# prashantraina/neural_raytracing

Hardware: NVIDIA B200
Metric: rays_per_sec (higher is better)
Workload: dtype f16

## Files before the change

### neural_raytracing_b200/csrc/nrt_tc.cu

```cuda
#include <stdlib.h>

#include "tc_core.cuh"
#include "camera_math.cuh"

namespace tc {

template <int IN, int LAT, int OUT>
struct IoPlain {
  const float* x; const float* latent; float* out; int out_act;
  __device__ __forceinline__ void load(int64_t m, float* v) const {
#pragma unroll
    for (int j = 0; j < IN; ++j) v[j] = __ldg(x + m * IN + j);
#pragma unroll
    for (int j = 0; j < LAT; ++j) v[IN + j] = __ldg(latent + m * LAT + j);
  }
  __device__ __forceinline__ void store(int64_t m, const float* o) const {
#pragma unroll
    for (int j = 0; j < OUT; ++j) {
      float v = o[j];
      if (out_act == NRT_OUT_SIGMOID) v = 1.0f / (1.0f + __expf(-v));
      else if (out_act == NRT_OUT_SOFTPLUS) v = v > 20.0f ? v : __logf(1.0f + __expf(v));
      else if (out_act == NRT_OUT_TANH) v = tanhf(v);
      out[m * OUT + j] = v;
    }
// ... 69 lines not shown
    }
  }
  __device__ __forceinline__ void load(int64_t m, float* v) const {
    const int64_t ray = ray_of(m, S, s_shift);
    if (lat32) {
      const float4* src = reinterpret_cast<const float4*>(latent) + (m >> 7) * (int64_t)(NLAT / 4 * 128) + (m & 127);
#pragma unroll
      for (int j = 0; j < NLAT / 4; ++j) {
        const float4 q = __ldg(src + j * 128);
        v[4 * j] = q.x; v[4 * j + 1] = q.y; v[4 * j + 2] = q.z; v[4 * j + 3] = q.w;
      }
    } else {
      const uint4* src = reinterpret_cast<const uint4*>(latent) + (m >> 7) * (int64_t)(NLAT / 8 * 128) + (m & 127);
#pragma unroll
      for (int j = 0; j < NLAT / 8; ++j) {
        const uint4 q = __ldg(src + j * 128);
        const uint32_t w[4] = {q.x, q.y, q.z, q.w};
#pragma unroll
        for (int e = 0; e < 4; ++e) {
          if (fmt == 0) {
            v[8 * j + 2 * e] = Elem<0>::back((uint16_t)(w[e] & 0xffff)); v[8 * j + 2 * e + 1] = Elem<0>::back((uint16_t)(w[e] >> 16));
          } else {
            v[8 * j + 2 * e] = Elem<1>::back((uint16_t)(w[e] & 0xffff)); v[8 * j + 2 * e + 1] = Elem<1>::back((uint16_t)(w[e] >> 16));
          }
        }
      }
    }
    const int view = dir_and_view(ray, v + NLAT);
#pragma unroll
    for (int j = 0; j < LD; ++j) v[NLAT + 3 + j] = __ldg(light_code + (int64_t)view * LD + j);
  }
  static constexpr int kPackedPairs = PACKED ? NLAT / 2 : 0;
  __device__ __forceinline__ void load_packed(int64_t m, uint32_t* w, float* v) const {
    const int64_t ray = ray_of(m, S, s_shift);
    const uint4* src = reinterpret_cast<const uint4*>(latent) + (m >> 7) * (int64_t)(NLAT / 8 * 128) + (m & 127);
#pragma unroll
    for (int j = 0; j < NLAT / 8; ++j) {
      const uint4 q = __ldg(src + j * 128);
      w[4 * j] = q.x; w[4 * j + 1] = q.y; w[4 * j + 2] = q.z; w[4 * j + 3] = q.w;
    }
    const int view = dir_and_view(ray, v + NLAT);
#pragma unroll
    for (int j = 0; j < LD; ++j) v[NLAT + 3 + j] = __ldg(light_code + (int64_t)view * LD + j);
  }
  __device__ __forceinline__ void store(int64_t m, const float* o) const {
#pragma unroll
    for (int j = 0; j < 3; ++j) {
      float v = o[j];
      if (out_act == NRT_OUT_SIGMOID) v = 1.0f / (1.0f + __expf(-v));
      else if (out_act == NRT_OUT_TANH) v = tanhf(v);
      rgb[m * 3 + j] = v;
    }
  }
};

static long long* g_dbg_timeline = nullptr;
extern "C" void nrtdbg_set_timeline(long long* dev_buf) { g_dbg_timeline = dev_buf; }

#ifndef NRT_SPH_MAX
#define NRT_SPH_MAX 128
#endif
constexpr int kSphMax = NRT_SPH_MAX;
__device__ __forceinline__ float* sph_table() {
  __shared__ __align__(16) float tab[kSphMax * 13];
  return tab;
}
__device__ __forceinline__ void sph_fill(const SdfDev& sd) {
  if (sd.n > kSphMax) return;
  float* tab = sph_table();
  for (int e = threadIdx.x; e < sd.n * 13; e += blockDim.x) {
    const int i = e / 13, k = e - i * 13;
    float v;
    if (k == 12) v = __ldg(sd.radii + i);
    else {
// ... 149 lines not shown
  __device__ __forceinline__ void store(int64_t m, const float* o) const {
    float p[3];
    point(m, p);
    val[m] = sphere_smin_fast<true>(sd, p[0], p[1], p[2]) + o[0];
  }
};
__global__ void k_scan_argmin(const float* __restrict__ val, const float* __restrict__ rays, int64_t R, int n1, double step,
                              int32_t* __restrict__ best_idx, float* __restrict__ best_pos, float* __restrict__ min_val) {
  const int lane = threadIdx.x & 31;
  const int64_t r = ((int64_t)blockIdx.x * blockDim.x + threadIdx.x) >> 5;
  if (r >= R) return;
  const float* v = val + r * n1;
  float best = 3.0e38f;
  int idx = 0x7fffffff;
  for (int k = lane; k < n1; k += 32) {
    const float x = v[k];
    if (x < best) { best = x; idx = k; }
  }
  for (int o = 16; o > 0; o >>= 1) {
    const float ob = __shfl_xor_sync(0xffffffffu, best, o);
    const int oi = __shfl_xor_sync(0xffffffffu, idx, o);
    if (ob < best || (ob == best && oi < idx)) { best = ob; idx = oi; }
  }
  if (lane == 0) {
    best_idx[r] = idx;
    if (min_val) min_val[r] = best;
    const float tb = __fmul_rn((float)idx, (float)step);
    for (int j = 0; j < 3; ++j) best_pos[r * 3 + j] = __fadd_rn(rays[r * 6 + j], __fmul_rn(tb, rays[r * 6 + 3 + j]));
  }
}

template <class NET, class IO, int FMT, class SV = NoSave>
static int launch(const void* blob, const IO& io, int64_t M, cudaStream_t st, int tag = TAG_TC_MLP, SV sv = SV{}) {
  const size_t bytes = (size_t)NET::SMEM_BYTES + 256;
  auto kern = k_mlp_tc<NET, IO, FMT, SV>;
  NRT_CUDA(cudaFuncSetAttribute(kern, cudaFuncAttributeMaxDynamicSharedMemorySize, (int)bytes));
  const int64_t ntiles = (M + 127) / 128;
  const int grid = (int)std::min<int64_t>((ntiles + NET::NSLOT - 1) / NET::NSLOT, (int64_t)nrt_sm_count());
  NrtProfScope _ps(tag, st);
  kern<<<grid, NET::threads(NET::WPS), bytes, st>>>(reinterpret_cast<const uint8_t*>(blob) + NET::BLOB_OFF, io, M, g_dbg_timeline, sv);
  NRT_CUDA(cudaGetLastError());
  return NRT_OK;
}

using NetNerfFirst = Net<3, 0, 16, 128, 5, 3, 65, NRT_ACT_LEAKY_RELU>;
using NetNerfFirstR = Net<3, 0, 16, 128, 5, 3, 65, NRT_ACT_LEAKY_RELU, (NRT_BIAS_MMA & 4) != 0>;
using NetNerfSecondPT = Net<70, 0, 16, 64, 8, 3, 3, NRT_ACT_LEAKY_RELU>;
using NetNerfSecondLE = Net<115, 0, 16, 64, 8, 3, 3, NRT_ACT_LEAKY_RELU>;
using NetNeuralBsdf = Net<3, 0, 64, 96, 6, 3, 3, NRT_ACT_LEAKY_RELU>;
using NetOcc = Net<5, 0, 16, 64, 8, 3, 1, NRT_ACT_LEAKY_RELU>;
using NetPlainFirst = Net<3, 32, 16, 32, 5, 3, 33, NRT_ACT_LEAKY_RELU>;
using NetPlainSecond = Net<2, 64, 16, 32, 5, 3, 3, NRT_ACT_LEAKY_RELU>;
using NetSdfShift = Net<3, 0, 32, 128, 8, 3, 1, NRT_ACT_SOFTPLUS>;

template <class NET>
static bool matches(const MlpDev& d) {
  return d.in_size == NET::IN && d.latent == NET::LAT && d.freqs == NET::F && d.hidden == NET::H && d.L == NET::L &&
         d.skip == NET::SKIP && d.out == NET::OUT && d.act == NET::ACT;
}
template <class NET>
static bool matches(const nrt_mlp_t& m) {
  return m.in_size == NET::IN && m.latent_size == NET::LAT && m.freqs == NET::F && m.hidden == NET::H && m.num_layers == NET::L &&
         m.skip == NET::SKIP && m.out_size == NET::OUT && m.act == NET::ACT;
}

}

using namespace tc;

static int fmt_of(int prec) { return prec == NRT_PREC_BF16 ? 1 : 0; }

extern "C" int64_t nrt_mlp_tc_blob_bytes(const nrt_mlp_t* m, int prec) {
  NRT_REQUIRE(m != nullptr, "mlp descriptor is NULL");
  NRT_REQUIRE(prec == NRT_PREC_F16 || prec == NRT_PREC_BF16, "nrt_mlp_tc_blob_bytes: prec must be F16 or BF16");
  NRT_REQUIRE(m->num_layers >= 1 && m->num_layers <= NRT_MAX_LAYERS && m->hidden % 16 == 0, "unsupported MLP shape");
  if (matches<NetNerfFirst>(*m)) return (int64_t)NetNerfFirstR::BLOB_OFF + NetNerfFirstR::Y.bytes;
  const Layout y = make_layout(m->in_size, m->latent_size, m->freqs, m->hidden, m->num_layers, m->skip, m->out_size);
  return (int64_t)y.bytes;
}

extern "C" int nrt_mlp_pack_tc(const nrt_mlp_t* m, int prec, void* blob_out, void* stream) {
// ... 234 lines not shown
```

### neural_raytracing_b200/csrc/tc_core.cuh

```cuda
#pragma once
#include <cuda_bf16.h>
#include <cuda_fp16.h>

#include <algorithm>
#include <type_traits>

#include "nrt_common.cuh"

namespace tc {

constexpr int kMaxOps = NRT_MAX_LAYERS + 3;

struct Layout {
  int split, XR, KRAW, KE, KX, KPH, FP, NOP;
  int n_ops;
  int opN[kMaxOps], opK[kMaxOps];
  int op_off[kMaxOps];
  int w_elems;
  int bias_off[kMaxOps];
  int bias_floats;
  int wout_f32_off;
  int basis_f32_off;
  int bytes;
};
// ... 673 lines not shown
          for (int i = 0; i < 8; ++i) q[i] = fmaf(q[i], u[i], 9.974489612e-01f);
#pragma unroll
          for (int i = 0; i < 8; ++i) a[i] = fmaf(q[i], u[i], fmaxf(a[i], 0.0f));
        } else {
#pragma unroll
          for (int i = 0; i < 8; ++i) u[i] = lg2_approx(1.0f + u[i]);
#pragma unroll
          for (int i = 0; i < 8; ++i) a[i] = fmaf(0.6931471805599453f, u[i], fmaxf(a[i], 0.0f));
        }
      } else {
#pragma unroll
        for (int i = 0; i < 8; ++i) a[i] = fmaxf(a[i], 0.01f * a[i]);
      }
#pragma unroll
      for (int i = 0; i < 8; ++i) {
        const float4 w = *reinterpret_cast<const float4*>(wout + (32 * c + 8 * g + i) * 4);
        o[0] = fmaf(a[i], w.x, o[0]);
        if constexpr (OUT > 1) o[1] = fmaf(a[i], w.y, o[1]);
        if constexpr (OUT > 2) o[2] = fmaf(a[i], w.z, o[2]);
        if constexpr (OUT > 3) o[3] = fmaf(a[i], w.w, o[3]);
      }
      if constexpr (SAVE) {
#pragma unroll
        for (int i = 0; i < 4; ++i) pk[4 * g + i] = Elem<FMT>::pack(a[2 * i], a[2 * i + 1]);
      }
    }
    if constexpr (SAVE) {
      save_cols<16>(save_row, 32 * c, pk);
      mask_ptr[(int64_t)c * mask_stride] = sign_mask32(pk);
    }
    if (c + 1 < NC) tc_wait_ld();
  }
  if constexpr (SAVE) save_row[tile_elem(H)] = one16<FMT>();
}

template <int ACT, int FMT, int H>
__device__ __forceinline__ void convert_row_savef32(uint32_t dD, uint32_t aU, float* __restrict__ acts, int64_t stride) {
  constexpr int NC = H / 32;
  uint32_t buf[2][32];
  TmemIO<32>::ld(dD, buf[0]);
  tc_wait_ld();
#pragma unroll
  for (int c = 0; c < NC; ++c) {
    if (c + 1 < NC) TmemIO<32>::ld(dD + 32 * (c + 1), buf[(c + 1) & 1]);
    uint32_t pk[16];
    convert32<ACT, FMT>(buf[c & 1], pk);
    TmemIO<16>::st(aU + 16 * c, pk);
    if (acts != nullptr) {
#pragma unroll
      for (int i = 0; i < 16; ++i) {
        acts[(int64_t)(32 * c + 2 * i) * stride] = Elem<FMT>::back((uint16_t)(pk[i] & 0xffffu));
        acts[(int64_t)(32 * c + 2 * i + 1) * stride] = Elem<FMT>::back((uint16_t)(pk[i] >> 16));
      }
    }
    if (c + 1 < NC) tc_wait_ld();
  }
}
template <int ACT, int FMT, int H, int OUT>
__device__ __forceinline__ void convert_row_out_savef32(uint32_t dD, const float* __restrict__ wout, float* __restrict__ o,
                                                        float* __restrict__ acts, int64_t stride) {
  constexpr int NC = H / 32;
  uint32_t buf[2][32];
  TmemIO<32>::ld(dD, buf[0]);
  tc_wait_ld();
#pragma unroll
  for (int c = 0; c < NC; ++c) {
// ... 158 lines not shown
  __syncwarp();
}
template <class NET, int FMT, int PART = 0, bool BMMA = false, int ZLO = 0>
__device__ __forceinline__ void issue_stage_dyn(int st, uint32_t b_addr, uint32_t dD, uint32_t aU, uint32_t aE,
                                                uint64_t* done_bar) {
#define NRT_STAGE_CASE(S) case S: if constexpr (S < NET::STAGES && (PART == 0 || S >= 2)) issue_stage<NET, FMT, S, PART, BMMA, ZLO>(b_addr, dD, aU, aE, done_bar); break;
  switch (st) {
    NRT_STAGE_CASE(0) NRT_STAGE_CASE(1) NRT_STAGE_CASE(2) NRT_STAGE_CASE(3) NRT_STAGE_CASE(4) NRT_STAGE_CASE(5)
    NRT_STAGE_CASE(6) NRT_STAGE_CASE(7) NRT_STAGE_CASE(8) NRT_STAGE_CASE(9) NRT_STAGE_CASE(10) NRT_STAGE_CASE(11)
    NRT_STAGE_CASE(12) NRT_STAGE_CASE(13) NRT_STAGE_CASE(14) NRT_STAGE_CASE(15) NRT_STAGE_CASE(16) NRT_STAGE_CASE(17)
    NRT_STAGE_CASE(18) NRT_STAGE_CASE(19) NRT_STAGE_CASE(20) NRT_STAGE_CASE(21) NRT_STAGE_CASE(22)
    default: break;
  }
#undef NRT_STAGE_CASE
}
__device__ __forceinline__ void stream_op(uint8_t* dst, const uint8_t* src, uint32_t bytes, uint64_t* bar) {
  mbar_expect_tx(bar, bytes);
  for (uint32_t off = 0; off < bytes; off += 32768u) bulk_g2s(dst + off, src + off, min(32768u, bytes - off), bar);
}

template <class T, class = void> struct PackedPairsOf { static constexpr int value = 0; };
template <class T> struct PackedPairsOf<T, std::void_t<decltype(T::kPackedPairs)>> { static constexpr int value = T::kPackedPairs; };
template <class T, class = void> struct HasCtaInit : std::false_type {};
template <class T> struct HasCtaInit<T, std::void_t<decltype(&T::cta_init)>> : std::true_type {};
template <class T, class = void> struct IsIterative : std::false_type {};
template <class T> struct IsIterative<T, std::void_t<typename T::State>> : std::true_type {};
struct NoState {};
template <class T, class = void> struct StateOf { using type = NoState; };
template <class T> struct StateOf<T, std::void_t<typename T::State>> { using type = typename T::State; };

__device__ __forceinline__ void named_bar_sync(int id, int nthreads) {
  asm volatile("bar.sync %0, %1;" ::"r"(id), "r"(nthreads) : "memory");
}

#ifdef NRT_MAXNREG
#define NRT_KMLP_BOUNDS(T) __maxnreg__(((65536 / (T)) / 8 * 8) > 255 ? 255 : ((65536 / (T)) / 8 * 8))
#else
#define NRT_KMLP_BOUNDS(T) __launch_bounds__(T, 1)
#endif
template <class NET, class IO, int FMT, class SV = NoSave, int WPS = NET::WPS>
__global__ void NRT_KMLP_BOUNDS(NET::threads(WPS))
k_mlp_tc(const uint8_t* __restrict__ blob, IO io, int64_t M, long long* __restrict__ dbg, SV sv = SV{}) {
  constexpr int EPI = WPS * 32;
  static_assert(NET::FITS_TMEM, "network does not fit in TMEM");
  static_assert(NET::FITS_SMEM, "stage buffers do not fit in shared memory");
  constexpr int kDbgIt0 = 4, kDbgIts = 4;
  auto stamp = [&](int it, int st, int slot, int k) {
    if (dbg != nullptr && slot < 2 && blockIdx.x == 0 && it >= kDbgIt0 && it < kDbgIt0 + kDbgIts)
      dbg[(((it - kDbgIt0) * NET::STAGES + st) * 2 + slot) * 8 + k] = clock64();
  };
  using E = Elem<FMT>;
  constexpr Layout Y = NET::Y;
  constexpr int H = NET::H, IN = NET::IN, LAT = NET::LAT, F = NET::F, L = NET::L;
  constexpr int NSLOT = NET::NSLOT;
  extern __shared__ __align__(128) uint8_t smem[];
  constexpr bool STREAM = NET::STREAM;
  uint16_t* sW = reinterpret_cast<uint16_t*>(smem);
  const float* sBias = reinterpret_cast<const float*>(smem + (STREAM ? (size_t)NSLOT * 2 * NET::MAXOP : (size_t)Y.w_elems * 2));
  __shared__ __align__(8) uint64_t bar_w;
  __shared__ __align__(8) uint64_t bar_wfull[3][2];
  __shared__ uint32_t s_opoff[NET::STAGES], s_opbytes[NET::STAGES];
  __shared__ __align__(8) uint64_t bar_ready[3];
  __shared__ __align__(8) uint64_t bar_ready_a[3];
  __shared__ __align__(8) uint64_t bar_done[3];
  constexpr bool KSPLIT = NET::KSPLIT && WPS == 4 && !SV::kOn && !SV::kF32;
#ifndef NRT_SOFTPLUS_FULLROW
#define NRT_SOFTPLUS_FULLROW 0
#endif
#ifndef NRT_SOFTPLUS_PIPE
#define NRT_SOFTPLUS_PIPE 1
#endif
  constexpr bool kPipeRow = NRT_SOFTPLUS_PIPE != 0 && SoftplusOf<IO>::value != 0 && NET::ACT == NRT_ACT_SOFTPLUS && !KSPLIT &&
                            !SV::kOn && !SV::kF32;
  constexpr bool kFullRow = NRT_SOFTPLUS_FULLROW != 0 && !kPipeRow && NET::ACT == NRT_ACT_SOFTPLUS && !KSPLIT && !SV::kOn && !SV::kF32;
  __shared__ uint32_t tmem_base_s;
  __shared__ uint32_t s_bias[NET::STAGES];
  constexpr bool ITER = IsIterative<IO>::value;
  constexpr bool BMMA = NET::BIAS_MMA && !KSPLIT && WPS == 4 && !SV::kOn && !SV::kF32;
  static_assert(BMMA || !NET::BIAS_ROWS, "the render layout has no fp32 biases to pre-load");
  constexpr int kPP = (!ITER && !NET::SPLIT && !SV::kOn && !SV::kF32 && LAT == 0 && NET::ACT == NRT_ACT_LEAKY_RELU) ? PackedPairsOf<IO>::value : 0;
  constexpr int ZLO = (NRT_BIAS_MMA & 2) ? 2 * kPP / 16 : 0;
  __shared__ volatile uint32_t s_slot_live[3];
  __shared__ uint32_t s_warp_live[3][4];

  const int tid = threadIdx.x;
  const int warp = tid >> 5;
  constexpr bool SELF = NET::SELF;
  const int mma_id = SELF ? -1 : warp - NET::NWG * WPS;
  const bool is_mma_warp = SELF ? warp == 0 : mma_id == 0;
  __shared__ uint32_t s_issue_lock;
  const int64_t ntiles = (M + 127) / 128;
  if constexpr (HasCtaInit<IO>::value) io.cta_init();
  if (tid < NET::STAGES) {
    s_bias[tid] = (uint32_t)Y.bias_off[tid];
    s_opoff[tid] = (uint32_t)Y.op_off[tid] * 2;
    s_opbytes[tid] = (uint32_t)(Y.opN[tid] * Y.opK[tid] * 2);
  }

  if (tid == 0) {
    s_slot_live[0] = 1; s_slot_live[1] = 1; s_slot_live[2] = 1;
    s_issue_lock = 0;
    mbar_init(&bar_w, 1);
    for (int s = 0; s < 3; ++s) {
      mbar_init(&bar_ready[s], EPI); mbar_init(&bar_done[s], 1); mbar_init(&bar_ready_a[s], EPI);
      mbar_init(&bar_wfull[s][0], 1); mbar_init(&bar_wfull[s][1], 1);
    }
    asm volatile("fence.mbarrier_init.release.cluster;" ::: "memory");
  }
  __syncthreads();
  if (is_mma_warp) {
    asm volatile("tcgen05.alloc.cta_group::1.sync.aligned.shared::cta.b32 [%0], 512;" ::"r"(smem_u32(&tmem_base_s)) : "memory");
    asm volatile("tcgen05.relinquish_alloc_permit.cta_group::1.sync.aligned;" ::: "memory");
    if ((tid & 31) == 0) {
      if (STREAM) {
        mbar_expect_tx(&bar_w, (uint32_t)NET::BIAS_BYTES);
        bulk_g2s(smem + (size_t)NSLOT * 2 * NET::MAXOP, blob + (size_t)Y.w_elems * 2, (uint32_t)NET::BIAS_BYTES, &bar_w);
      } else {
        mbar_expect_tx(&bar_w, (uint32_t)Y.bytes);
        constexpr uint32_t kChunk = 32768;
        for (uint32_t off = 0; off < (uint32_t)Y.bytes; off += kChunk) {
          const uint32_t n = min(kChunk, (uint32_t)Y.bytes - off);
          bulk_g2s(smem + off, blob + off, n, &bar_w);
        }
      }
    }
  }
  tc_fence_before();
  __syncthreads();
  tc_fence_after();
  if (tmem_base_s != 0u) __trap();
  constexpr uint32_t tmem = 0u;
  if constexpr (BMMA) {
    if (warp < 4) {
      const uint32_t one = (uint32_t)one16<FMT>();
      const uint32_t r[8] = {one | (one << 16), one, 0u, 0u, 0u, 0u, 0u, 0u};
      TmemIO<8>::st(tmem + ((uint32_t)(warp * 32) << 16) + (uint32_t)NET::ONES_COL, r);
      tc_wait_st();
    }
    tc_fence_before();
    __syncthreads();
    tc_fence_after();
  }
  mbar_wait(&bar_w, 0);

  if (mma_id >= 0) {
    constexpr int NMMA = NET::NMMA;
    constexpr bool OWN = NMMA == NSLOT;
    auto mine = [&](int slot) { return slot % (NMMA > 0 ? NMMA : 1) == mma_id; };
#ifndef NRT_MMA_ALTERNATE
#define NRT_MMA_ALTERNATE 0
#endif
    constexpr bool ALT = NRT_MMA_ALTERNATE != 0 && !OWN && NSLOT == 2 && !KSPLIT;
    int turn = 0;
    bool live[3];
    auto is_ready = [&](int slot, uint64_t* bar, uint32_t parity) {
      if constexpr (OWN) { mbar_wait(bar, parity); return true; }
      else if constexpr (ALT) {
        if (slot != turn && live[turn]) return false;
        mbar_wait(bar, parity);
        turn = slot ^ 1;
        return true;
      }
      else return mbar_test(bar, parity);
    };
    const uint32_t sW_addr = smem_u32(sW);
    int st[3] = {NET::FIRST_STAGE, NET::FIRST_STAGE, NET::FIRST_STAGE};
    uint32_t n_ready[3] = {0, 0, 0};
    uint32_t n_ready_a[3] = {0, 0, 0};
    bool half_issued[3] = {false, false, false};
    int64_t tile[3] = {(int64_t)blockIdx.x * NSLOT, (int64_t)blockIdx.x * NSLOT + 1, (int64_t)blockIdx.x * NSLOT + 2};
    live[0] = mine(0) && (ITER || tile[0] < ntiles);
    live[1] = NSLOT > 1 && mine(1) && (ITER || tile[1] < ntiles);
    live[2] = NSLOT > 2 && mine(2) && (ITER || tile[2] < ntiles);
    int it_dbg[3] = {0, 0, 0};
    uint32_t n_issued[3] = {0, 0, 0};
    if (STREAM) {
#pragma unroll
      for (int slot = 0; slot < NSLOT; ++slot)
        if (live[slot] && elect_one())
          stream_op(smem + (size_t)(slot * 2) * NET::MAXOP, blob + s_opoff[NET::FIRST_STAGE], s_opbytes[NET::FIRST_STAGE],
                    &bar_wfull[slot][0]);
      __syncwarp();
    }
    while (live[0] || live[1] || live[2]) {
      bool progressed = false;
#pragma unroll
      for (int slot = 0; slot < NSLOT; ++slot) {
        if (!live[slot]) continue;
        if constexpr (KSPLIT) {
          if (st[slot] >= 2 && !half_issued[slot]) {
            if (!is_ready(slot, &bar_ready_a[slot], n_ready_a[slot] & 1)) continue;
            progressed = true;
            n_ready_a[slot]++;
            half_issued[slot] = true;
            tc_fence_after();
            const uint32_t base = tmem + slot * NET::COLS;
            uint32_t b_addr = sW_addr;
            if (STREAM) {
              const uint32_t b = n_issued[slot] & 1;
              mbar_wait(&bar_wfull[slot][b], (n_issued[slot] >> 1) & 1);
              b_addr = sW_addr + (uint32_t)((slot * 2 + b) * NET::MAXOP);
            }
            if ((tid & 31) == 0) stamp(it_dbg[slot], st[slot], slot, 0);
            issue_stage_dyn<NET, FMT, 1>(st[slot], b_addr, base, base + NET::DC, base + NET::DC + NET::UC, &bar_done[slot]);
            continue;
          }
        }
        if (!is_ready(slot, &bar_ready[slot], n_ready[slot] & 1)) continue;
        progressed = true;
        n_ready[slot]++;
        tc_fence_after();
        if constexpr (ITER) {
          if (st[slot] == NET::FIRST_STAGE && s_slot_live[slot] == 0) {
            live[slot] = false;
            if (STREAM) mbar_wait(&bar_wfull[slot][n_issued[slot] & 1], (n_issued[slot] >> 1) & 1);
            continue;
          }
        }
        if ((tid & 31) == 0) stamp(it_dbg[slot], st[slot], slot, 1);
        const uint32_t base = tmem + slot * NET::COLS;
        uint32_t b_addr = sW_addr;
        if (STREAM) {
          const uint32_t b = n_issued[slot] & 1;
          mbar_wait(&bar_wfull[slot][b], (n_issued[slot] >> 1) & 1);
          b_addr = sW_addr + (uint32_t)((slot * 2 + b) * NET::MAXOP);
          if ((tid & 31) == 0) stamp(it_dbg[slot], st[slot], slot, 0);
        }
        if (KSPLIT && half_issued[slot]) {
          half_issued[slot] = false;
          issue_stage_dyn<NET, FMT, 2>(st[slot], b_addr, base, base + NET::DC, base + NET::DC + NET::UC, &bar_done[slot]);
        } else {
          issue_stage_dyn<NET, FMT, 0, BMMA, ZLO>(st[slot], b_addr, base, base + NET::DC, base + NET::DC + NET::UC, &bar_done[slot]);
        }
        if ((tid & 31) == 0) stamp(it_dbg[slot], st[slot], slot, 2);
        if (++st[slot] == NET::END_STAGE) {
          st[slot] = NET::FIRST_STAGE;
          it_dbg[slot]++;
          if constexpr (!ITER) {
            tile[slot] += (int64_t)gridDim.x * NSLOT;
            live[slot] = tile[slot] < ntiles;
          }
        }
        if (STREAM) {
          n_issued[slot]++;
          if (live[slot] && elect_one()) {
            const uint32_t nb = n_issued[slot] & 1;
            stream_op(smem + (size_t)(slot * 2 + nb) * NET::MAXOP, blob + s_opoff[st[slot]], s_opbytes[st[slot]],
                      &bar_wfull[slot][nb]);
          }
          __syncwarp();
        }
      }
#ifndef NRT_MMA_POLL_SLEEP_NS
#define NRT_MMA_POLL_SLEEP_NS 0
#endif
      if (NRT_MMA_POLL_SLEEP_NS > 0 && !progressed) __nanosleep(NRT_MMA_POLL_SLEEP_NS);
    }
  } else {
    const int slot = warp / WPS;
    const int half = (WPS == 8) ? ((warp >> 2) & 1) : 0;
    const bool primary = half == 0;
    const int lane_row = (warp & 3) * 32 + (tid & 31);
    constexpr int HW = (WPS == 8) ? H / 2 : H;
    if (slot < NSLOT) {
      const uint32_t lane_off = ((uint32_t)((warp & 3) * 32)) << 16;
      const uint32_t base = tmem + slot * NET::COLS + lane_off;
      const uint32_t dD = base, aU = base + NET::DC, aE = base + NET::DC + NET::UC;
      uint32_t n_done = 0;
      int it_dbg = 0;
#ifndef NRT_DBG_LANE
#define NRT_DBG_LANE 0
#endif
      auto estamp = [&](int st, int k) { if (lane_row == NRT_DBG_LANE) stamp(it_dbg, st, slot, k); };
      typename StateOf<IO>::type state;
      if constexpr (ITER) io.init(state);
      const bool leader = SELF && (warp % WPS) == 0;
      int st_mma = NET::FIRST_STAGE;
      uint32_t n_ready_l = 0, n_issued_l = 0;
      const uint32_t sW_addr_l = smem_u32(sW);
      if constexpr (SELF) {
        if (leader) {
          if (elect_one())
            stream_op(smem + (size_t)(slot * 2) * NET::MAXOP, blob + s_opoff[NET::FIRST_STAGE], s_opbytes[NET::FIRST_STAGE],
                      &bar_wfull[slot][0]);
          __syncwarp();
        }
      }
      auto self_issue = [&]() {
        if constexpr (SELF) {
          if (leader) {
            mbar_wait(&bar_ready[slot], n_ready_l & 1); n_ready_l++;
            const uint32_t b = n_issued_l & 1;
            mbar_wait(&bar_wfull[slot][b], (n_issued_l >> 1) & 1);
            if ((tid & 31) == 0) {
              while (atomicCAS(&s_issue_lock, 0u, 1u) != 0u) __nanosleep(64);
            }
            __syncwarp();
            tc_fence_after();
            if ((tid & 31) == 0) stamp(it_dbg, st_mma, slot, 1);
            const uint32_t base0 = tmem + slot * NET::COLS;
            issue_stage_dyn<NET, FMT>(st_mma, sW_addr_l + (uint32_t)((slot * 2 + b) * NET::MAXOP), base0, base0 + NET::DC,
                                      base0 + NET::DC + NET::UC, &bar_done[slot]);
            if ((tid & 31) == 0) {
              stamp(it_dbg, st_mma, slot, 2);
              __threadfence_block();
              atomicExch(&s_issue_lock, 0u);
            }
            if (++st_mma == NET::END_STAGE) st_mma = NET::FIRST_STAGE;
            n_issued_l++;
            if (elect_one()) {
              const uint32_t nb = n_issued_l & 1;
              stream_op(smem + (size_t)(slot * 2 + nb) * NET::MAXOP, blob + s_opoff[st_mma], s_opbytes[st_mma], &bar_wfull[slot][nb]);
            }
            __syncwarp();
          }
        }
      };
      auto self_drain = [&]() {
        if constexpr (SELF) {
          if (leader) mbar_wait(&bar_wfull[slot][n_issued_l & 1], (n_issued_l >> 1) & 1);
        }
      };
#ifndef NRT_SLOT_STAGGER
#define NRT_SLOT_STAGGER 900
#endif
      if (NRT_SLOT_STAGGER > 0 && slot > 0) {
        const long long t_start = clock64();
        while (clock64() - t_start < (long long)slot * NRT_SLOT_STAGGER) {}
      }
      for (int64_t t0 = (int64_t)blockIdx.x * NSLOT;; t0 += (int64_t)gridDim.x * NSLOT, ++it_dbg) {
        int64_t m = 0;
        bool valid;
        float x[IN + LAT];
        uint32_t pw[kPP > 0 ? kPP : 1];
        if constexpr (ITER) {
          valid = primary ? io.next(state, x) : false;
          const unsigned bal = __ballot_sync(0xffffffffu, valid);
          if (primary && (tid & 31) == 0) s_warp_live[slot][warp & 3] = bal;
          named_bar_sync(1 + slot, EPI);
          const bool any = (s_warp_live[slot][0] | s_warp_live[slot][1] | s_warp_live[slot][2] | s_warp_live[slot][3]) != 0;
          if (!any) {
            if (lane_row == 0) s_slot_live[slot] = 0;
            mbar_arrive(&bar_ready[slot]);
            self_drain();
            break;
          }
        } else {
          const int64_t tile = t0 + slot;
          if (tile >= ntiles) { self_drain(); break; }
          m = tile * 128 + lane_row;
          valid = m < M;
          if constexpr (kPP > 0) {
            if (valid && primary) io.load_packed(m, pw, x);
          } else {
            if (valid && primary) io.load(m, x);
          }
        }
        if (!primary) {
          if constexpr (!NET::ENC_CUDA) {
            mbar_arrive(&bar_ready[slot]);
            mbar_wait(&bar_done[slot], n_done & 1); n_done++;
          }
          mbar_arrive(&bar_ready[slot]);
          self_issue();
        } else {
        uint32_t ex[NET::XR / 2];
        {
          if (!valid) {
#pragma unroll
            for (int j = 0; j < IN + LAT; ++j) x[j] = 0.0f;
          }
          uint32_t ax[NET::KX / 2];
#pragma unroll
          for (int j = 0; j < NET::KX / 2; ++j) { ax[j] = 0; ex[j] = 0; }
          if constexpr (NET::SPLIT) {
            uint16_t v[16];
#pragma unroll
            for (int j = 0; j < 16; ++j) v[j] = 0;
            uint16_t a[2 * IN];
#pragma unroll
            for (int j = 0; j < IN; ++j) {
              const uint16_t hi = E::cvt(x[j]);
              const uint16_t lo = E::cvt(x[j] - E::back(hi));
              v[j] = hi; v[IN + j] = lo; v[2 * IN + j] = hi;
              const float ax_ = act_fast<NET::ACT>(x[j]);
              const uint16_t ahi = E::cvt(ax_);
              a[j] = ahi; a[IN + j] = E::cvt(ax_ - E::back(ahi));
            }
            if constexpr (NET::BIAS_ROWS) {
#pragma unroll
              for (int t = 0; t < 3; ++t) v[NET::BR.row + t] = one16<FMT>();
            }
#pragma unroll
            for (int j = 0; j < 8; ++j) ax[j] = (uint32_t)v[2 * j] | ((uint32_t)v[2 * j + 1] << 16);
#pragma unroll
            for (int j = 0; j < IN; ++j) ex[j] = (uint32_t)a[2 * j] | ((uint32_t)a[2 * j + 1] << 16);
            if constexpr (NET::BIAS_ROWS) {
#pragma unroll
              for (int t = 0; t < 3; ++t) ex[(NET::BR.row + t) / 2] |= (uint32_t)one16<FMT>() << (16 * ((NET::BR.row + t) & 1));
            }
// ... 19 lines not shown
            }
            if constexpr (NET::INPLACE) { tmem_store<NET::XR / 2>(aE, ax); tmem_store<NET::XR / 2>(aU, lx); }
            else { tmem_store<NET::XR / 2>(aU, ax); tmem_store<NET::XR / 2>(aE, lx); }
          }
          if constexpr (SV::kOn) {
            static_assert(!ITER, "activation tiles are saved by the tile policies only");
            uint16_t* rr = tile_row_ptr(sv.enc_raw, m >> 7, NET::KE + kTileRowsExtra, lane_row);
            uint16_t* ra = tile_row_ptr(sv.enc_act, m >> 7, NET::KE + kTileRowsExtra, lane_row);
            save_cols<NET::KX / 2>(rr, 0, ax);
            if constexpr (!NET::INPLACE) save_cols<NET::XR / 2>(ra, 0, ex);
            rr[tile_elem(NET::KE)] = one16<FMT>();
            ra[tile_elem(NET::KE)] = one16<FMT>();
          }
          if constexpr (LAT > 0) {
            uint32_t lr[LAT / 2], la[LAT / 2];
#pragma unroll
            for (int j = 0; j < LAT / 2; ++j) {
              lr[j] = E::pack(x[IN + 2 * j], x[IN + 2 * j + 1]);
              la[j] = E::pack(act_fast<NET::ACT>(x[IN + 2 * j]), act_fast<NET::ACT>(x[IN + 2 * j + 1]));
            }
            tmem_store<LAT / 2>(aU + (NET::XR + 2 * F) / 2, lr);
            tmem_store<LAT / 2>(aE + (NET::XR + 2 * F) / 2, la);
            if constexpr (SV::kOn) {
              save_cols<LAT / 2>(tile_row_ptr(sv.enc_raw, m >> 7, NET::KE + kTileRowsExtra, lane_row), NET::XR + 2 * F, lr);
              save_cols<LAT / 2>(tile_row_ptr(sv.enc_act, m >> 7, NET::KE + kTileRowsExtra, lane_row), NET::XR + 2 * F, la);
            }
          }
          if constexpr (!NET::ENC_CUDA) {
            tc_wait_st();
            tc_fence_before();
            mbar_arrive(&bar_ready[slot]);
          }
        }
        {
          uint32_t ph[F];
          if constexpr (NET::ENC_CUDA) {
            const float* sB = sBias + Y.basis_f32_off;
#pragma unroll
            for (int f = 0; f < F; ++f) {
              float p = x[0] * sB[f];
#pragma unroll
              for (int j = 1; j < IN; ++j) p = fmaf(x[j], sB[j * NET::FP + f], p);
              ph[f] = __float_as_uint(p);
            }
          } else {
            mbar_wait(&bar_done[slot], n_done & 1); n_done++;
            tc_fence_after();
            tmem_load<F>(dD, ph);
            tc_wait_ld();
            if constexpr (!NET::INPLACE) tmem_store<NET::XR / 2>(aE, ex);
          }
          if constexpr (!BMMA) preload_bias<H>(dD, sBias + s_bias[1]);
          uint32_t sr[F / 2], cr[F / 2], sa[F / 2], ca[F / 2];
#pragma unroll
          for (int j = 0; j < F / 2; ++j) {
            float s0, c0, s1, c1;
            sincos_fast(__uint_as_float(ph[2 * j]), &s0, &c0);
            sincos_fast(__uint_as_float(ph[2 * j + 1]), &s1, &c1);
            sr[j] = E::pack(s0, s1); cr[j] = E::pack(c0, c1);
            sa[j] = E::pack(act_fast<NET::ACT>(s0), act_fast<NET::ACT>(s1));
            ca[j] = E::pack(act_fast<NET::ACT>(c0), act_fast<NET::ACT>(c1));
          }
          if constexpr (NET::INPLACE) {
            tmem_store<F / 2>(aE + NET::XR / 2, sr);
            tmem_store<F / 2>(aE + NET::XR / 2 + F / 2, cr);
          } else {
            tmem_store<F / 2>(aU + NET::XR / 2, sr);
// ... 55 lines not shown
            long long* d = nullptr;
            if (dbg != nullptr && lane_row == 0 && slot < 2 && blockIdx.x == 0 && it_dbg >= kDbgIt0 && it_dbg < kDbgIt0 + kDbgIts)
              d = dbg + (((it_dbg - kDbgIt0) * NET::STAGES + 2 + st) * 2 + slot) * 8;
            convert_row_split<NET::ACT, FMT, HW>(dD, aU, &bar_ready_a[slot], &bar_ready[slot], pre, d ? d + 5 : nullptr,
                                                 d ? d + 6 : nullptr);
            estamp(2 + st, 7);
          } else {
          if constexpr (SV::kOn)
            convert_row<NET::ACT, FMT, HW, true>(dD + coff, aU + coff / 2,
                tile_row_ptr(sv.acts, (int64_t)st * sv.ntiles + (m >> 7), H + kTileRowsExtra, lane_row), coff, primary ? H : -1,
                sv.masks + (int64_t)st * (H / 32) * (sv.ntiles * 128) + m, sv.ntiles * 128);
          else if constexpr (SV::kF32)
            convert_row_savef32<NET::ACT, FMT, HW>(dD + coff, aU + coff / 2,
                                                   valid ? sv.acts + ((int64_t)st * H) * sv.M + m : nullptr, sv.M);
          else if constexpr (kPipeRow) {
            long long* d = nullptr;
#ifdef NRT_DBG_CONV
            if (dbg != nullptr && lane_row == NRT_DBG_LANE && slot < 2 && blockIdx.x == 0 && it_dbg >= kDbgIt0 && it_dbg < kDbgIt0 + kDbgIts)
              d = dbg + (((it_dbg - kDbgIt0) * NET::STAGES + 2 + st) * 2 + slot) * 8 + 3;
#endif
            convert_row_pipe<FMT, HW, SoftplusOf<IO>::value>(dD + coff, aU + coff / 2, pre, d);
          }
          else if constexpr (kFullRow)
            convert_row_full<NET::ACT, FMT, HW>(dD + coff, aU + coff / 2, pre);
          else
            convert_row<NET::ACT, FMT, HW>(dD + coff, aU + coff / 2);
          if constexpr (!(kFullRow || kPipeRow) || SV::kOn || SV::kF32) pre();
          estamp(2 + st, 6);
          tc_wait_st();
          tc_fence_before();
          mbar_arrive(&bar_ready[slot]);
          estamp(2 + st, 7);
          self_issue();
          }
        }
        if (!primary) {
          mbar_wait(&bar_done[slot], n_done & 1); n_done++;
          tc_fence_after();
          tc_fence_before();
        } else if constexpr (NET::FUSE_OUT) {
          mbar_wait(&bar_done[slot], n_done & 1); n_done++;
          tc_fence_after();
          float o[NET::OUT];
#pragma unroll
          for (int j = 0; j < NET::OUT; ++j) o[j] = sBias[s_bias[NET::STAGES - 1] + j];
          if constexpr (SV::kOn)
            convert_row_out<NET::ACT, FMT, H, NET::OUT, true>(dD, sBias + Y.wout_f32_off, o,
                tile_row_ptr(sv.acts, (int64_t)L * sv.ntiles + (m >> 7), H + kTileRowsExtra, lane_row),
                sv.masks + (int64_t)L * (H / 32) * (sv.ntiles * 128) + m, sv.ntiles * 128);
          else if constexpr (SV::kF32)
            convert_row_out_savef32<NET::ACT, FMT, H, NET::OUT>(dD, sBias + Y.wout_f32_off, o,
                                                                  valid ? sv.acts + ((int64_t)L * H) * sv.M + m : nullptr, sv.M);
          else
            convert_row_out<NET::ACT, FMT, H, NET::OUT, false, kPipeRow || (NRT_SOFTPLUS_POLY != 0)>(dD, sBias + Y.wout_f32_off, o);
          if constexpr (ITER) { if (valid) io.consume(state, o); }
          else { if (valid) io.store(m, o); }
          tc_fence_before();
        } else {
          mbar_wait(&bar_done[slot], n_done & 1); n_done++;
          tc_fence_after();
          constexpr int OC = (NET::OUT + 7) / 8 * 8;
          uint32_t acc[OC];
          tmem_load<OC>(dD, acc);
          tc_wait_ld();
          float o[NET::OUT];
#pragma unroll
          for (int j = 0; j < NET::OUT; ++j) o[j] = __uint_as_float(acc[j]);
          if constexpr (ITER) { if (valid) io.consume(state, o); }
          else { if (valid) io.store(m, o); }
          tc_fence_before();
        }
      }
      if constexpr (ITER) { if (primary) io.finish(state); }
    }
  }
  tc_fence_before();
  __syncthreads();
  if (is_mma_warp) asm volatile("tcgen05.dealloc.cta_group::1.sync.aligned.b32 %0, 512;" ::"r"(tmem) : "memory");
}


}
```

Measured before the change: 13.17 million.

## Pipeline next-tile input staging and sin/cos encoding across tile boundaries

Adds a pipelined tile-boundary path for the NeRF second MLP. The next tile's packed latents are prefetched into per-slot shared-memory stages with cp.async, written to tensor memory after the last hidden stage, and the first MMA stage is issued early against a new inputs barrier. The sin/cos encoding of the next tile is interleaved with the current tile's fused output layer. The goal is to hide global-load latency and MMA idle gaps at tile boundaries, at the cost of more shared memory, extra mbarriers and a more intricate synchronisation protocol.

```diff
diff --git a/neural_raytracing_b200/csrc/nrt_tc.cu b/neural_raytracing_b200/csrc/nrt_tc.cu
--- a/neural_raytracing_b200/csrc/nrt_tc.cu
+++ b/neural_raytracing_b200/csrc/nrt_tc.cu
@@ -125,14 +125,33 @@
   }
   static constexpr int kPackedPairs = PACKED ? NLAT / 2 : 0;
   __device__ __forceinline__ void load_packed(int64_t m, uint32_t* w, float* v) const {
-    const int64_t ray = ray_of(m, S, s_shift);
     const uint4* src = reinterpret_cast<const uint4*>(latent) + (m >> 7) * (int64_t)(NLAT / 8 * 128) + (m & 127);
 #pragma unroll
     for (int j = 0; j < NLAT / 8; ++j) {
       const uint4 q = __ldg(src + j * 128);
       w[4 * j] = q.x; w[4 * j + 1] = q.y; w[4 * j + 2] = q.z; w[4 * j + 3] = q.w;
     }
-    const int view = dir_and_view(ray, v + NLAT);
+    load_dir_light(m, v);
+  }
+  __device__ __forceinline__ void prefetch_packed(int64_t m, uint4* stage, float* v) const {
+    const uint4* src = reinterpret_cast<const uint4*>(latent) + (m >> 7) * (int64_t)(NLAT / 8 * 128) + (m & 127);
+    const uint32_t dst = (uint32_t)__cvta_generic_to_shared(stage + (m & 127));
+#pragma unroll
+    for (int j = 0; j < NLAT / 8; ++j)
+      asm volatile("cp.async.cg.shared.global [%0], [%1], 16;" ::"r"(dst + j * 128 * 16), "l"(src + j * 128) : "memory");
+    asm volatile("cp.async.commit_group;" ::: "memory");
+    load_dir_light(m, v);
+  }
+  __device__ __forceinline__ static void load_staged(const uint4* stage, int row, uint32_t* w) {
+    asm volatile("cp.async.wait_all;" ::: "memory");
+#pragma unroll
+    for (int j = 0; j < NLAT / 8; ++j) {
+      const uint4 q = stage[j * 128 + row];
+      w[4 * j] = q.x; w[4 * j + 1] = q.y; w[4 * j + 2] = q.z; w[4 * j + 3] = q.w;
+    }
+  }
+  __device__ __forceinline__ void load_dir_light(int64_t m, float* v) const {
+    const int view = dir_and_view(ray_of(m, S, s_shift), v + NLAT);
 #pragma unroll
     for (int j = 0; j < LD; ++j) v[NLAT + 3 + j] = __ldg(light_code + (int64_t)view * LD + j);
   }
@@ -348,7 +367,7 @@
 
 template <class NET, class IO, int FMT, class SV = NoSave>
 static int launch(const void* blob, const IO& io, int64_t M, cudaStream_t st, int tag = TAG_TC_MLP, SV sv = SV{}) {
-  const size_t bytes = (size_t)NET::SMEM_BYTES + 256;
+  const size_t bytes = (size_t)TileBoundary<NET, IO, SV, NET::WPS>::SMEM_BYTES + 256;
   auto kern = k_mlp_tc<NET, IO, FMT, SV>;
   NRT_CUDA(cudaFuncSetAttribute(kern, cudaFuncAttributeMaxDynamicSharedMemorySize, (int)bytes));
   const int64_t ntiles = (M + 127) / 128;
@@ -363,6 +382,10 @@
 using NetNerfFirstR = Net<3, 0, 16, 128, 5, 3, 65, NRT_ACT_LEAKY_RELU, (NRT_BIAS_MMA & 4) != 0>;
 using NetNerfSecondPT = Net<70, 0, 16, 64, 8, 3, 3, NRT_ACT_LEAKY_RELU>;
 using NetNerfSecondLE = Net<115, 0, 16, 64, 8, 3, 3, NRT_ACT_LEAKY_RELU>;
+template <class IO> using NerfSecondPTBoundary = TileBoundary<NetNerfSecondPT, IO, NoSave, NetNerfSecondPT::WPS>;
+static_assert(NerfSecondPTBoundary<IoNerfSecond<64, 3, true>>::PIPE && NerfSecondPTBoundary<IoNerfSecond<64, 3, true, true>>::PIPE &&
+              NerfSecondPTBoundary<IoNerfSecond<64, 3, true>>::SMEM_BYTES == 154496 + 3 * 16384 &&
+              154496 + 3 * 16384 <= kSmemBudget, "NeRFLE.second: pipelined tile boundary");
 using NetNeuralBsdf = Net<3, 0, 64, 96, 6, 3, 3, NRT_ACT_LEAKY_RELU>;
 using NetOcc = Net<5, 0, 16, 64, 8, 3, 1, NRT_ACT_LEAKY_RELU>;
 using NetPlainFirst = Net<3, 32, 16, 32, 5, 3, 33, NRT_ACT_LEAKY_RELU>;
diff --git a/neural_raytracing_b200/csrc/tc_core.cuh b/neural_raytracing_b200/csrc/tc_core.cuh
--- a/neural_raytracing_b200/csrc/tc_core.cuh
+++ b/neural_raytracing_b200/csrc/tc_core.cuh
@@ -729,6 +729,20 @@
     if (c + 1 < NC) tc_wait_ld();
   }
   if constexpr (SAVE) save_row[tile_elem(H)] = one16<FMT>();
+}
+template <int H, int OUT>
+__device__ __forceinline__ void out_layer_regs(const uint32_t* __restrict__ acc, const float* __restrict__ wout, float* __restrict__ o) {
+  static_assert(OUT <= 4, "fused output layer");
+#pragma unroll
+  for (int k = 0; k < H; ++k) {
+    float a = __uint_as_float(acc[k]);
+    a = fmaxf(a, 0.01f * a);
+    const float4 w = *reinterpret_cast<const float4*>(wout + k * 4);
+    o[0] = fmaf(a, w.x, o[0]);
+    if constexpr (OUT > 1) o[1] = fmaf(a, w.y, o[1]);
+    if constexpr (OUT > 2) o[2] = fmaf(a, w.z, o[2]);
+    if constexpr (OUT > 3) o[3] = fmaf(a, w.w, o[3]);
+  }
 }
 
 template <int ACT, int FMT, int H>
@@ -953,6 +967,23 @@
 __device__ __forceinline__ void named_bar_sync(int id, int nthreads) {
   asm volatile("bar.sync %0, %1;" ::"r"(id), "r"(nthreads) : "memory");
 }
+
+template <class NET, class IO, class SV, int WPS>
+struct TileBoundary {
+  static constexpr bool ITER = IsIterative<IO>::value;
+  static constexpr int PP = (!ITER && !NET::SPLIT && !SV::kOn && !SV::kF32 && NET::LAT == 0 && NET::ACT == NRT_ACT_LEAKY_RELU)
+                                ? PackedPairsOf<IO>::value : 0;
+  static constexpr int ZLO = (NRT_BIAS_MMA & 2) ? 2 * PP / 16 : 0;
+  static constexpr int LAST = NET::END_STAGE - 1;
+  static constexpr int STAGE_OFF = (NET::Y.bytes + 127) / 128 * 128;
+  static constexpr int STAGE_BYTES = 128 * PP * 4;
+  static constexpr bool PIPE = NET::INPLACE && !NET::ENC_CUDA && NET::FUSE_OUT && !NET::STREAM && NET::BIAS_MMA &&
+                               !NET::KSPLIT && WPS == 4 && PP > 0 && PP % 4 == 0 && NET::Y.opK[LAST] == NET::H &&
+                               8 * ZLO >= NET::H / 2 && NET::XR / 2 + NET::FP <= NET::EC &&
+                               STAGE_OFF + NET::NSLOT * STAGE_BYTES <= kSmemBudget;
+  static constexpr int SMEM_BYTES = PIPE ? STAGE_OFF + NET::NSLOT * STAGE_BYTES : NET::SMEM_BYTES;
+  static_assert(SMEM_BYTES <= kSmemBudget, "shared memory");
+};
 
 #ifdef NRT_MAXNREG
 #define NRT_KMLP_BOUNDS(T) __maxnreg__(((65536 / (T)) / 8 * 8) > 255 ? 255 : ((65536 / (T)) / 8 * 8))
@@ -999,8 +1030,12 @@
   constexpr bool ITER = IsIterative<IO>::value;
   constexpr bool BMMA = NET::BIAS_MMA && !KSPLIT && WPS == 4 && !SV::kOn && !SV::kF32;
   static_assert(BMMA || !NET::BIAS_ROWS, "the render layout has no fp32 biases to pre-load");
-  constexpr int kPP = (!ITER && !NET::SPLIT && !SV::kOn && !SV::kF32 && LAT == 0 && NET::ACT == NRT_ACT_LEAKY_RELU) ? PackedPairsOf<IO>::value : 0;
-  constexpr int ZLO = (NRT_BIAS_MMA & 2) ? 2 * kPP / 16 : 0;
+  using TB = TileBoundary<NET, IO, SV, WPS>;
+  constexpr int kPP = TB::PP;
+  constexpr int ZLO = TB::ZLO;
+  constexpr bool PIPE = TB::PIPE;
+  __shared__ __align__(8) uint64_t bar_inputs[3];
+  __shared__ __align__(8) uint64_t bar_phase[3];
   __shared__ volatile uint32_t s_slot_live[3];
   __shared__ uint32_t s_warp_live[3][4];
 
@@ -1025,6 +1060,7 @@
     for (int s = 0; s < 3; ++s) {
       mbar_init(&bar_ready[s], EPI); mbar_init(&bar_done[s], 1); mbar_init(&bar_ready_a[s], EPI);
       mbar_init(&bar_wfull[s][0], 1); mbar_init(&bar_wfull[s][1], 1);
+      mbar_init(&bar_inputs[s], EPI); mbar_init(&bar_phase[s], 1);
     }
     asm volatile("fence.mbarrier_init.release.cluster;" ::: "memory");
   }
@@ -1087,6 +1123,7 @@
     const uint32_t sW_addr = smem_u32(sW);
     int st[3] = {NET::FIRST_STAGE, NET::FIRST_STAGE, NET::FIRST_STAGE};
     uint32_t n_ready[3] = {0, 0, 0};
+    uint32_t n_inputs[3] = {0, 0, 0};
     uint32_t n_ready_a[3] = {0, 0, 0};
     bool half_issued[3] = {false, false, false};
     int64_t tile[3] = {(int64_t)blockIdx.x * NSLOT, (int64_t)blockIdx.x * NSLOT + 1, (int64_t)blockIdx.x * NSLOT + 2};
@@ -1127,9 +1164,14 @@
             continue;
           }
         }
-        if (!is_ready(slot, &bar_ready[slot], n_ready[slot] & 1)) continue;
+        if (PIPE && st[slot] == 0) {
+          if (!is_ready(slot, &bar_inputs[slot], n_inputs[slot] & 1)) continue;
+          n_inputs[slot]++;
+        } else {
+          if (!is_ready(slot, &bar_ready[slot], n_ready[slot] & 1)) continue;
+          n_ready[slot]++;
+        }
         progressed = true;
-        n_ready[slot]++;
         tc_fence_after();
         if constexpr (ITER) {
           if (st[slot] == NET::FIRST_STAGE && s_slot_live[slot] == 0) {
@@ -1150,6 +1192,9 @@
         if (KSPLIT && half_issued[slot]) {
           half_issued[slot] = false;
           issue_stage_dyn<NET, FMT, 2>(st[slot], b_addr, base, base + NET::DC, base + NET::DC + NET::UC, &bar_done[slot]);
+        } else if (PIPE && st[slot] == 0) {
+          issue_stage<NET, FMT, 0, 0, BMMA, ZLO>(b_addr, base + NET::DC + NET::UC + NET::XR / 2, base + NET::DC,
+                                                 base + NET::DC + NET::UC, &bar_phase[slot]);
         } else {
           issue_stage_dyn<NET, FMT, 0, BMMA, ZLO>(st[slot], b_addr, base, base + NET::DC, base + NET::DC + NET::UC, &bar_done[slot]);
         }
@@ -1187,8 +1232,47 @@
       const uint32_t lane_off = ((uint32_t)((warp & 3) * 32)) << 16;
       const uint32_t base = tmem + slot * NET::COLS + lane_off;
       const uint32_t dD = base, aU = base + NET::DC, aE = base + NET::DC + NET::UC;
-      uint32_t n_done = 0;
+      uint32_t n_done = 0, n_phase = 0;
       int it_dbg = 0;
+      uint4* lat_stage = reinterpret_cast<uint4*>(smem + TB::STAGE_OFF + (size_t)slot * TB::STAGE_BYTES);
+      auto put_packed = [&](bool v, const uint32_t* w, const float* xs) {
+        uint32_t ax[NET::XR / 2], lx[NET::XR / 2];
+#pragma unroll
+        for (int j = 0; j < NET::XR / 2; ++j) { ax[j] = 0; lx[j] = 0; }
+#pragma unroll
+        for (int j = 0; j < (IN + 1) / 2; ++j) {
+          if (j < kPP) { ax[j] = v ? w[j] : 0u; continue; }
+          const float xa = v ? xs[2 * j] : 0.0f, xb = (v && 2 * j + 1 < IN) ? xs[2 * j + 1 < IN ? 2 * j + 1 : 0] : 0.0f;
+          ax[j] = E::pack(xa, xb);
+          const float ha = E::back((uint16_t)(ax[j] & 0xffffu)), hb = E::back((uint16_t)(ax[j] >> 16));
+          lx[j] = E::pack(xa - ha, xb - hb);
+        }
+        tmem_store<NET::XR / 2>(aE, ax);
+        tmem_store<NET::XR / 2 - 8 * ZLO>(aU + 8 * ZLO, lx + 8 * ZLO);
+      };
+      auto sincos_in_place = [&]() {
+        uint32_t ph[F];
+        mbar_wait(&bar_phase[slot], n_phase & 1); n_phase++;
+        tc_fence_after();
+        tmem_load<F>(aE + NET::XR / 2, ph);
+        tc_wait_ld();
+#pragma unroll
+        for (int q = 0; q < F / 8; ++q) {
+          uint32_t sr[4], cr[4];
+#pragma unroll
+          for (int j = 0; j < 4; ++j) {
+            float s0, c0, s1, c1;
+            sincos_fast(__uint_as_float(ph[8 * q + 2 * j]), &s0, &c0);
+            sincos_fast(__uint_as_float(ph[8 * q + 2 * j + 1]), &s1, &c1);
+            sr[j] = E::pack(s0, s1); cr[j] = E::pack(c0, c1);
+          }
+          tmem_store<4>(aE + NET::XR / 2 + 4 * q, sr);
+          tmem_store<4>(aE + NET::XR / 2 + F / 2 + 4 * q, cr);
+        }
+        tc_wait_st();
+        tc_fence_before();
+        mbar_arrive(&bar_ready[slot]);
+      };
 #ifndef NRT_DBG_LANE
 #define NRT_DBG_LANE 0
 #endif
@@ -1252,6 +1336,10 @@
       for (int64_t t0 = (int64_t)blockIdx.x * NSLOT;; t0 += (int64_t)gridDim.x * NSLOT, ++it_dbg) {
         int64_t m = 0;
         bool valid;
+        const bool inputs_in_place = PIPE && t0 != (int64_t)blockIdx.x * NSLOT;
+        const int64_t next_tile = t0 + slot + (int64_t)gridDim.x * NSLOT;
+        const bool has_next = PIPE && next_tile < ntiles;
+        const bool valid_next = has_next && next_tile * 128 + lane_row < M;
         float x[IN + LAT];
         uint32_t pw[kPP > 0 ? kPP : 1];
         if constexpr (ITER) {
@@ -1272,7 +1360,7 @@
           m = tile * 128 + lane_row;
           valid = m < M;
           if constexpr (kPP > 0) {
-            if (valid && primary) io.load_packed(m, pw, x);
+            if (valid && primary && !inputs_in_place) io.load_packed(m, pw, x);
           } else {
             if (valid && primary) io.load(m, x);
           }
@@ -1286,7 +1374,14 @@
           self_issue();
         } else {
         uint32_t ex[NET::XR / 2];
-        {
+        if constexpr (PIPE) {
+          if (!inputs_in_place) {
+            put_packed(valid, pw, x);
+            tc_wait_st();
+            tc_fence_before();
+            mbar_arrive(&bar_inputs[slot]);
+          }
+        } else {
           if (!valid) {
 #pragma unroll
             for (int j = 0; j < IN + LAT; ++j) x[j] = 0.0f;
@@ -1372,7 +1467,10 @@
             mbar_arrive(&bar_ready[slot]);
           }
         }
-        {
+        if constexpr (PIPE) {
+          if (!inputs_in_place) sincos_in_place();
+          if (valid_next) io.prefetch_packed(next_tile * 128 + lane_row, lat_stage, x);
+        } else {
           uint32_t ph[F];
           if constexpr (NET::ENC_CUDA) {
             const float* sB = sBias + Y.basis_f32_off;
@@ -1494,6 +1592,15 @@
           mbar_arrive(&bar_ready[slot]);
           estamp(2 + st, 7);
           self_issue();
+          if constexpr (PIPE) {
+            if (st == NHID - 1 && has_next) {
+              if (valid_next) io.load_staged(lat_stage, lane_row, pw);
+              put_packed(valid_next, pw, x);
+              tc_wait_st();
+              tc_fence_before();
+              mbar_arrive(&bar_inputs[slot]);
+            }
+          }
           }
         }
         if (!primary) {
@@ -1503,6 +1610,7 @@
         } else if constexpr (NET::FUSE_OUT) {
           mbar_wait(&bar_done[slot], n_done & 1); n_done++;
           tc_fence_after();
+          estamp(NET::STAGES - 1, 4);
           float o[NET::OUT];
 #pragma unroll
           for (int j = 0; j < NET::OUT; ++j) o[j] = sBias[s_bias[NET::STAGES - 1] + j];
@@ -1513,7 +1621,21 @@
           else if constexpr (SV::kF32)
             convert_row_out_savef32<NET::ACT, FMT, H, NET::OUT>(dD, sBias + Y.wout_f32_off, o,
                                                                   valid ? sv.acts + ((int64_t)L * H) * sv.M + m : nullptr, sv.M);
-          else
+          else if constexpr (PIPE) {
+            constexpr int kHeld = 40;
+            static_assert(kHeld > 0 && kHeld <= H && kHeld % 8 == 0, "output-layer columns held across sin / cos");
+            if constexpr (kHeld < H) {
+              uint32_t acc0[H - kHeld];
+              tmem_load<H - kHeld>(dD, acc0);
+              tc_wait_ld();
+              out_layer_regs<H - kHeld, NET::OUT>(acc0, sBias + Y.wout_f32_off, o);
+            }
+            uint32_t acc[kHeld];
+            tmem_load<kHeld>(dD + H - kHeld, acc);
+            tc_wait_ld();
+            if (has_next) sincos_in_place();
+            out_layer_regs<kHeld, NET::OUT>(acc, sBias + Y.wout_f32_off + (H - kHeld) * 4, o);
+          } else
             convert_row_out<NET::ACT, FMT, H, NET::OUT, false, kPipeRow || (NRT_SOFTPLUS_POLY != 0)>(dD, sBias + Y.wout_f32_off, o);
           if constexpr (ITER) { if (valid) io.consume(state, o); }
           else { if (valid) io.store(m, o); }
```

Result: no change. 13.28 million (median of 6 runs) (+0.8%).
